# svg-project/Sparse-VideoGen

Hardware: AMD Instinct MI355X
Metric: attn_tflops_svg1_block_sparse (higher is better)
Workload: dtype bf16; 1 GPU; HunyuanVideo T2V hy720p SVG1 sparse layer-call: sample_mse(64 rows) + band attention with fused head placement, cfg=1 H=24 D=128 F=33 P=3600 ctx=256 prompt=64 S=119056 band=15616 density=0.2456; parallelism=single, variant=0, heads=alt

## Files before the change

### include/svg_attn.h

```cpp
#ifndef SVG_ATTN_H_
#define SVG_ATTN_H_

#include <stddef.h>
#include <stdint.h>

#ifdef __cplusplus
extern "C" {
#endif

#define SVG_DTYPE_BF16 0
#define SVG_DTYPE_F16 1
#define SVG_DTYPE_F32 2

#define SVG_OK 0
#define SVG_ERR_BAD_ARG (-1)
#define SVG_ERR_UNSUPPORTED (-2)
#define SVG_ERR_WORKSPACE (-3)
#define SVG_ERR_LAUNCH (-4)

#define SVG_ABI_VERSION 4
int svg_abi_version(void);

const char* svg_strerror(int code);
int svg_last_hip_error(void);
// ... 175 lines not shown
typedef struct svg_prologue_segment {
    const void* q_in;
    const void* k_in;
    const void* v_in;
    int32_t rows;
    int32_t norm_kind;
    const void* q_weight;
    const void* q_bias;
    const void* k_weight;
    const void* k_bias;
    float eps;
} svg_prologue_segment_t;

int svg_qk_norm_rope_transpose_joint(const svg_prologue_segment_t* seg, int32_t n_seg, void* q_out, void* k_out, void* v_out,
                                     int32_t bsz, int32_t H, int32_t D, int32_t dtype, int32_t rope_kind, const float* cos_or_real,
                                     const float* sin_or_imag, int32_t rope_lo, int32_t rope_hi, float q_scale, void* stream);

int svg_rmsnorm_rope_transpose(const void* q_in, const void* k_in, const void* v_in, void* q_out, void* k_out, void* v_out, int32_t bsz,
                               int32_t H, int32_t S, int32_t D, int32_t dtype, const void* q_weight, const void* k_weight,
                               int32_t w_dtype, float eps, int32_t rope_kind, const float* cos_or_real, const float* sin_or_imag,
                               int32_t rope_lo, int32_t rope_hi, float q_scale, void* stream);

int svg_layernorm_forward(const void* x, void* y, const void* weight, const void* bias, int64_t M, int32_t N, int32_t x_dtype,
                          int32_t y_dtype, int32_t w_dtype, float eps, void* stream);
int svg_modulate_shift_forward(const void* x, void* y, const float* scale, const float* shift, int64_t M, int32_t N,
                               int64_t rows_per_batch, int32_t x_dtype, int32_t y_dtype, void* stream);
int svg_modulate_gate_residual_forward(const void* residual, const void* x, const float* gate, void* y, int64_t M, int32_t N,
                                       int64_t rows_per_batch, int32_t r_dtype, int32_t x_dtype, int32_t y_dtype,
                                       void* stream);
int svg_layernorm_modulate_forward(const void* x, void* y, const void* weight, const void* bias, const float* scale,
                                   const float* shift, int64_t M, int32_t N, int64_t rows_per_batch, int32_t x_dtype,
                                   int32_t y_dtype, int32_t w_dtype, float eps, void* stream);
int svg_rmsnorm_forward(const void* x, void* y, const void* weight, int64_t M, int32_t N, int32_t x_dtype, int32_t y_dtype,
                        int32_t w_dtype, float eps, void* stream);
int svg_layernorm_forward_ex(const void* x, void* y, const void* weight, const void* bias, int64_t M, int32_t N, int32_t x_dtype,
                             int32_t y_dtype, int32_t w_dtype, float eps, int32_t reference_padding, void* stream);
int svg_layernorm_modulate_forward_ex(const void* x, void* y, const void* weight, const void* bias, const float* scale,
                                      const float* shift, int64_t M, int32_t N, int64_t rows_per_batch, int32_t x_dtype,
                                      int32_t y_dtype, int32_t w_dtype, float eps, int32_t reference_padding, void* stream);

int svg_band_attention_switch(const void* q, const void* k, const void* v, void* o, int32_t BH, int32_t S, int32_t D,
                              int32_t dtype, float sm_scale, const svg_band_mask_t* mask, const svg_perm_desc_t* perm,
                              const svg_band_mask_t* alt_mask, const int32_t* use_alt_flag, void* stream);
int svg_band_attention_switch_strided(const void* q, const void* k, const void* v, void* o, int32_t BH, int32_t S, int32_t D,
                                      int32_t dtype, float sm_scale, const svg_band_mask_t* mask, const svg_perm_desc_t* perm,
                                      const svg_band_mask_t* alt_mask, const int32_t* use_alt_flag,
                                      const svg_attn_layout_t* layout, void* stream);
int svg_sample_mse_flagged(const void* q, const void* k, const void* v, const int64_t* rows, int32_t R, int32_t BH, int32_t S,
                           int32_t D, int32_t dtype, float sm_scale, const svg_profile_desc_t* prof, float* out_mse,
                           void* workspace, size_t workspace_bytes, const int32_t* skip_flag, void* stream);

size_t svg_band_attention_fp8_workspace_bytes(int32_t BH, int32_t S, int32_t D);
int svg_band_attention_fp8(const void* q, const void* k, const void* v, void* o, int32_t BH, int32_t S, int32_t D, int32_t dtype,
                           float sm_scale, const svg_band_mask_t* mask, const svg_perm_desc_t* perm, void* workspace,
                           size_t workspace_bytes, void* stream);
int svg_band_attention_fp8_stage(const void* q, const void* k, const void* v, void* o, int32_t BH, int32_t S, int32_t D, int32_t dtype,
                                 float sm_scale, const svg_band_mask_t* mask, const svg_perm_desc_t* perm, void* workspace,
                                 size_t workspace_bytes, int32_t stage, void* stream);

size_t svg_varblock_attention_fp8_workspace_bytes(int32_t Hq, int32_t Hkv, int32_t QB, int32_t KB, int32_t Sq, int32_t Skv, int32_t D);
int svg_varblock_attention_fp8(const void* q, const void* k, const void* v, void* o, int32_t Hq, int32_t Hkv, int32_t Sq, int32_t Skv,
                               int32_t D, int32_t dtype, float sm_scale, const uint8_t* block_map, const int32_t* q_sizes,
                               const int32_t* k_sizes, int32_t QB, int32_t KB, const int32_t* q_row_idx, const int32_t* kv_row_idx,
                               void* workspace, size_t workspace_bytes, void* stream);

int32_t svg_band_attention_notify_target(int32_t S, const svg_band_mask_t* mask);
int svg_band_attention_notify(const void* q, const void* k, const void* v, void* o, int32_t BH, int32_t S, int32_t D,
                              int32_t dtype, float sm_scale, const svg_band_mask_t* mask, const svg_perm_desc_t* perm,
                              int32_t* done_per_head, int32_t done_words, void* stream);
int svg_wait_counters(const int32_t* counters, int32_t n, int32_t target, void* stream);
int svg_wait_counters_deadline(const int32_t* counters, int32_t n, int32_t target, int32_t timeout_ms, int32_t* timed_out,
                               void* stream);
int32_t svg_band_attention_notify_layout(int32_t S, const svg_band_mask_t* mask, int32_t nseg, int32_t* row_bounds, int32_t* targets);
int svg_band_attention_notify_seg(const void* q, const void* k, const void* v, void* o, int32_t BH, int32_t S, int32_t D,
                                  int32_t dtype, float sm_scale, const svg_band_mask_t* mask, const svg_perm_desc_t* perm,
                                  int32_t* done, int32_t done_words, int32_t nseg, void* stream);
int svg_band_attention_prescaled_notify_seg(const void* q_scaled, const void* k, const void* v, void* o, int32_t BH, int32_t S,
                                            int32_t D, int32_t dtype, const svg_band_mask_t* mask, const svg_perm_desc_t* perm,
                                            int32_t* done, int32_t done_words, int32_t nseg, void* stream);

int32_t svg_band_queue_order(int32_t BH, int32_t S, const svg_band_mask_t* mask, int32_t* out, int32_t out_words);
int svg_debug_band_queue_cap(int32_t max_workgroups);
int64_t svg_debug_band_replays(int32_t reset);

int svg_debug_pp_trace(uint64_t* out104);

int svg_debug_clock_probe(const int32_t* stop_flag, uint64_t* out2, int32_t max_ms, void* stream);

int svg_debug_wg_trace(uint64_t* out, int32_t n_workgroups);

#ifdef __cplusplus
}
#endif
#endif
```

### sparse-videogen_amd/csrc/attention.hip

```cpp
#include <algorithm>
#include <atomic>
#include <mutex>

#include "attn_core.h"
#include "attn_m16.h"
#include "band_policy.h"

namespace svg {

template <typename T, int D, int NW>
__global__ __launch_bounds__(NW * 64, 2) void band_attn_kernel(typename BandPolicy<T, D, NW>::Params prm) {
    extern __shared__ __attribute__((aligned(16))) char smem[];
    attn_body<T, D, NW, BandPolicy<T, D, NW>>(prm, smem, nullptr);
}

template <typename T, int D>
__global__ __launch_bounds__(512, (D == 64 ? 4 : 2)) void band_attn_pp2_kernel(typename BandPolicy<T, D, 8>::Params prm) {
    extern __shared__ __attribute__((aligned(16))) char smem[];
    attn_body_pp2<T, D, BandPolicy<T, D, 8>, false, 0, false, D == 64>(prm, smem, nullptr);
}
template <typename T>
__global__ __launch_bounds__(512, 4) void band_attn_pp2_switch64_kernel(typename BandPolicy<T, 64, 8>::Params prm,
                                                                        typename BandPolicy<T, 64, 8>::Params prm_alt,
                                                                        const int32_t* __restrict__ flag) {
// ... 370 lines not shown
extern "C" int svg_wait_counters(const int32_t* counters, int32_t n, int32_t target, void* stream) {
    if (!counters || n <= 0) return SVG_ERR_BAD_ARG;
    hipLaunchKernelGGL(wait_counters_kernel, dim3(1), dim3(64), 0, (hipStream_t)stream, counters, n, target);
    return launch_status();
}

extern "C" int svg_wait_counters_deadline(const int32_t* counters, int32_t n, int32_t target, int32_t timeout_ms,
                                          int32_t* timed_out, void* stream) {
    if (!counters || n <= 0 || timeout_ms <= 0 || !timed_out) return SVG_ERR_BAD_ARG;
    hipLaunchKernelGGL(wait_counters_deadline_kernel, dim3(1), dim3(64), 0, (hipStream_t)stream, counters, n, target,
                       (long long)timeout_ms * 100000LL, timed_out);
    return launch_status();
}

static BandOpts switch_opts(const svg_band_mask_t* alt_mask, const int32_t* use_alt_flag) {
    BandOpts opts;
    opts.alt_mask = alt_mask, opts.use_alt = use_alt_flag;
    return opts;
}

extern "C" int svg_band_attention_switch(const void* q, const void* k, const void* v, void* o, int32_t BH, int32_t S, int32_t D,
                                         int32_t dtype, float sm_scale, const svg_band_mask_t* mask, const svg_perm_desc_t* perm,
                                         const svg_band_mask_t* alt_mask, const int32_t* use_alt_flag, void* stream) {
    if (!alt_mask || !use_alt_flag) return SVG_ERR_BAD_ARG;
    return band_dispatch(q, k, v, o, BH, S, D, dtype, sm_scale, mask, perm, kBandAuto, switch_opts(alt_mask, use_alt_flag), 0, nullptr,
                         stream);
}

extern "C" int svg_band_attention_switch_strided(const void* q, const void* k, const void* v, void* o, int32_t BH, int32_t S, int32_t D,
                                                 int32_t dtype, float sm_scale, const svg_band_mask_t* mask, const svg_perm_desc_t* perm,
                                                 const svg_band_mask_t* alt_mask, const int32_t* use_alt_flag,
                                                 const svg_attn_layout_t* layout, void* stream) {
    if (!layout || !alt_mask || !use_alt_flag) return SVG_ERR_BAD_ARG;
    BandOpts opts = switch_opts(alt_mask, use_alt_flag);
    opts.strided = true;
    return band_dispatch(q, k, v, o, BH, S, D, dtype, sm_scale, mask, perm, kBandAuto, opts, 0, layout, stream);
}

extern "C" int svg_band_attention_switch_prescaled(const void* q_scaled, const void* k, const void* v, void* o, int32_t BH, int32_t S,
                                                   int32_t D, int32_t dtype, const svg_band_mask_t* mask, const svg_perm_desc_t* perm,
                                                   const svg_band_mask_t* alt_mask, const int32_t* use_alt_flag, void* stream) {
    if (!alt_mask || !use_alt_flag) return SVG_ERR_BAD_ARG;
    BandOpts opts = switch_opts(alt_mask, use_alt_flag);
    opts.prescaled = true;
    return band_dispatch(q_scaled, k, v, o, BH, S, D, dtype, 1.f, mask, perm, kBandAuto, opts, 0, nullptr, stream);
}

extern "C" int32_t svg_band_queue_order(int32_t BH, int32_t S, const svg_band_mask_t* mask, int32_t* out, int32_t out_words) {
    if (!mask || BH <= 0 || S <= 0 || check_band_mask(S, mask, nullptr) != SVG_OK) return -1;
    using Pol = svg::BandPolicy<__bf16, 128, 8>;
    const auto p = svg::make_band_params<Pol, __bf16>(nullptr, nullptr, nullptr, nullptr, BH, S, 1.f, mask, nullptr);
    const BandQueue qd = svg::make_band_queue<Pol>(p);
    if (!out) return qd.n_items;
    int n = 0;
    for (int x = 0; x <= kNumXCD; ++x)
        for (unsigned i = 0;; ++i) {
            const int w = x < kNumXCD ? qd.item(x, i) : qd.tail_item(i);
            if (w < 0) break;
            if (3 * (n + 1) > out_words) return -1;
            int head, qt;
            qd.decode(w, head, qt);
            Pol::Ctx c;
            Pol::kv_schedule(p, c, qt);
            out[3 * n] = x, out[3 * n + 1] = head * p.nqt + qt, out[3 * n + 2] = c.nT;
            ++n;
        }
    return n;
}

extern "C" int svg_debug_band_queue_cap(int32_t max_workgroups) {
    if (max_workgroups < 0) return SVG_ERR_BAD_ARG;
    g_queue_cap.store(max_workgroups, std::memory_order_relaxed);
    return SVG_OK;
}

extern "C" int64_t svg_debug_band_replays(int32_t reset) {
    unsigned n = 0;
    if (hipDeviceSynchronize() != hipSuccess || hipMemcpyFromSymbol(&n, HIP_SYMBOL(g_band_replays), sizeof n) != hipSuccess) return -1;
    const unsigned zero = 0;
    if (reset && hipMemcpyToSymbol(HIP_SYMBOL(g_band_replays), &zero, sizeof zero) != hipSuccess) return -1;
    return (int64_t)n;
}

extern "C" int svg_debug_wg_trace(uint64_t* out, int n_workgroups) { return g_trace_reader(out, true, n_workgroups); }
extern "C" int svg_debug_pp_trace(uint64_t* out104) { return g_trace_reader(out104, false, 0); }
```

### sparse-videogen_amd/csrc/attn_m16.h

```cpp
#pragma once
#include "attn_core.h"

namespace svg {

template <typename T>
struct Mfma16;
template <>
struct Mfma16<__bf16> {
    static __device__ __forceinline__ f32x4 mfma(bf16x8 a, bf16x8 b, f32x4 c) { return __builtin_amdgcn_mfma_f32_16x16x32_bf16(a, b, c, 0, 0, 0); }
    static __device__ __forceinline__ f32x4 mfma_keep_c(bf16x8 a, bf16x8 b, const f32x4& c) {
        f32x4 d;
        asm volatile("v_mfma_f32_16x16x32_bf16 %0, %1, %2, %3" : "=&v"(d) : "v"(a), "v"(b), "v"(c));
        return d;
    }
};
template <>
struct Mfma16<_Float16> {
    static __device__ __forceinline__ f32x4 mfma(f16x8 a, f16x8 b, f32x4 c) { return __builtin_amdgcn_mfma_f32_16x16x32_f16(a, b, c, 0, 0, 0); }
    static __device__ __forceinline__ f32x4 mfma_keep_c(f16x8 a, f16x8 b, const f32x4& c) {
        f32x4 d;
        asm volatile("v_mfma_f32_16x16x32_f16 %0, %1, %2, %3" : "=&v"(d) : "v"(a), "v"(b), "v"(c));
        return d;
    }
};

constexpr int attn_m16_lds_bytes() { return attn_pp2_lds_bytes<128>(); }

template <int D>
struct KvImage16 {
    static constexpr int kImg = kBN * D * 2, kStage = 2 * kImg;
    static constexpr unsigned col_v(int lane) {
        return ((lane & 3) ^ ((unsigned)((lane >> 4) & 1) << 1)) * 16u;
    }
    static constexpr unsigned col_k(int lane) { return col_v(lane); }
    static constexpr int k_lane(int g4, int n16) { return (n16 << 6) | ((g4 ^ (((n16 >> 2) & 1) << 1)) << 4); }
    static constexpr int v_lane0(int g4, int n16) { return kImg + (4 * g4 + (n16 >> 2)) * 64 + (((g4 & 1) * 16) + 4 * (n16 & 3)) * 2; }
    static constexpr int k_off(int k_lane, int kblk, int ks) { return k_lane + ks * (kBN * 64) + kblk * 1024; }
    static constexpr int v_off(int v_lane0, int v_lane1, int kc, int db, int h) {
        return ((db & 1) ? v_lane1 : v_lane0) + (db >> 1) * (kBN * 64) + (32 * kc + 16 * h) * 64;
    }
    static __device__ __forceinline__ i16x8 kfrag(const char* st, int k_lane, int kblk, int ks) {
        return *(const i16x8*)(st + k_off(k_lane, kblk, ks));
    }
    static __device__ __forceinline__ i16x8 vfrag(const char* st, int v_lane0, int v_lane1, int kc, int db) {
        return lds_read_tr16x2(st + v_off(v_lane0, v_lane1, kc, db, 0), st + v_off(v_lane0, v_lane1, kc, db, 1));
    }
    static constexpr int k_read(int key, int c) { return k_off(k_lane(c & 3, key & 15), key >> 4, c >> 2); }
    static constexpr int v_read(int key, int d) {
        const int lane = 16 * ((key >> 2) & 3) + (d & 15), src = tr16_src_lane(lane, key & 3), vl0 = v_lane0(src >> 4, src & 15);
        return v_off(vl0, vl0 ^ 32, key >> 5, d >> 4, (key >> 4) & 1) + 2 * (lane & 3);
    }
};
static_assert(kv_image_consistent<KvImage16<64>, 64>() && kv_image_consistent<KvImage16<128>, 128>(),
              "KvImage16: DMA columns and fragment reads disagree");

__device__ __forceinline__ float quad_group_max(float x) {
    x = vmax2(x, __shfl_xor(x, 16));
    return vmax2(x, __shfl_xor(x, 32));
}
__device__ __forceinline__ float quad_group_sum(float x) {
    x += __shfl_xor(x, 16);
    return x + __shfl_xor(x, 32);
}

template <typename P, typename = void>
struct HasAddOnStore : std::false_type {};
template <typename P>
struct HasAddOnStore<P, std::void_t<decltype(&P::add_on_store)>> : std::true_type {};

template <typename T>
__device__ __forceinline__ u32x2 add_rounded16(u32x2 a, u32x2 b) {
    using E = Elt<T>;
    const typename E::v4 x = __builtin_bit_cast(typename E::v4, a), y = __builtin_bit_cast(typename E::v4, b);
    typename E::v4 s;
#pragma unroll
    for (int j = 0; j < 4; ++j) s[j] = E::from_float(E::to_float(x[j]) + E::to_float(y[j]));
    return __builtin_bit_cast(u32x2, s);
}

constexpr int kCheckEvery = 8;
template <typename T, typename P, bool TRACE = false, int ONEBAR = -1, bool PRE = false, bool SPEC = false>
__device__ __forceinline__ bool attn_m16_tile(const typename P::Params& prm, const typename P::Ctx& ctx, char* smem,
                                              int check_mask = kCheckEvery - 1, unsigned* replay_ctr = nullptr) {
    using E = Elt<T>;
    using M = Mfma16<T>;
    using V8 = typename E::v8;
    constexpr int D = 128;
    constexpr int NW = 8;
    constexpr int KS = D / 32;
    constexpr int NDB = D / 16;
    using Img = KvImage16<D>;
    constexpr int NS = 4;
    constexpr int kImg = Img::kImg, kStage = Img::kStage;
    constexpr int NP = 2;
    constexpr int kCarry = 8;
    constexpr int kPF = 8;
    constexpr bool kOneBar = ONEBAR < 0 ? P::kOneBarrier : (ONEBAR != 0);
    static_assert(P::kRowBlocks == 1 && !P::kPartialOut && !P::kFixup && P::kIntervalMask, "band / variable-block policy");
    constexpr bool MSUM = std::is_same_v<T, __bf16> && !PRE;
    constexpr float kBias = MSUM ? 10.f : 0.f;
    constexpr bool kSpec = SPEC && MSUM;
    static_assert(!(SPEC && TRACE) && (kCheckEvery & (kCheckEvery - 1)) == 0, "SPEC: product kernels; a power of two");

    unsigned long long wg_t0 = 0, wg_t2 = 0;
    if constexpr (TRACE) wg_t0 = __builtin_amdgcn_s_memtime();
    const int tid = threadIdx.x;
    const int lane = tid & 63;
    const int wave = wave_id();
    const int g4 = lane >> 4;
    const int n16 = lane & 15;
    const bool lagging = wave >= NW / 2;
    const int nT = ctx.nT;
    volatile int* const spec_word = (volatile int*)(smem + attn_m16_lds_bytes() + 8);

    const T* __restrict__ qb = P::q_base(prm, ctx);
    const T* __restrict__ kb_ = P::k_base(prm, ctx);
    const T* __restrict__ vb = P::v_base(prm, ctx);
    const unsigned lds0 = (unsigned)(size_t)smem;

    const int dma_kg = wave / 2;
    const int dma_db0 = (wave % 2) * NP;
    const int krow = 16 * dma_kg + (lane >> 2);
    typename P::KvCursor cur;
    P::kv_cursor_init(prm, ctx, cur, krow);
    const unsigned col_v = (unsigned)(dma_db0 * 64 + Img::col_v(lane));
    const unsigned lds_piece = lds0 + (unsigned)(dma_db0 * (kBN * 64) + dma_kg * 1024);
    int nphys = 0, nnext = 0;
    auto resolve = [&](int t, auto guard_c) {
        if constexpr (decltype(guard_c)::value) nnext = (t < nT) ? P::kv_phys(prm, ctx, cur, t, krow) : 0;
        else nnext = P::kv_phys(prm, ctx, cur, t, krow);
    };
    constexpr std::true_type kGuarded{};
    auto take = [&]() { nphys = nnext; };
    const unsigned k_rsb = (unsigned)P::k_rs(prm) * 2u, v_rsb = (unsigned)P::v_rs(prm) * 2u;
    auto dma_piece = [&](int t, auto j_c) {
        constexpr int j = decltype(j_c)::value;
        const unsigned st = __builtin_amdgcn_readfirstlane(lds_piece + (unsigned)((t % NS) * kStage) + j * (kBN * 64));
        const unsigned ko = __umul24((unsigned)nphys, k_rsb) + col_v;
        const unsigned vo = __umul24((unsigned)nphys, v_rsb) + col_v;
        lds_dma16_kv<kImg>(st, ko, vo, (const char*)kb_ + j * 64, (const char*)vb + j * 64);
    };
    auto dma_issue = [&](int t) {
        dma_piece(t, std::integral_constant<int, 0>{});
        dma_piece(t, std::integral_constant<int, 1>{});
    };
    const int dist = lagging ? 3 : 2;
    for (int t = 0; t < dist; ++t) {
        resolve(t, kGuarded);
        take();
        if (t < nT) dma_issue(t);
    }
    resolve(dist, kGuarded);

    int q_log[2];
    V8 qf[2][KS];
    int m_a0[2], m_b0[2];
    unsigned m_alen[2], m_blen[2];
#pragma unroll
    for (int rb = 0; rb < 2; ++rb) {
        const int row_in_wg = wave * 32 + rb * 16 + n16;
        const int qp = P::q_phys(prm, ctx, row_in_wg);
        q_log[rb] = P::q_logical(ctx, row_in_wg);
        const T* qrow = qb + (size_t)(qp >= 0 ? qp : 0) * P::q_rs(prm) + g4 * 8;
#pragma unroll
        for (int ks = 0; ks < KS; ++ks) qf[rb][ks] = *(const V8*)(qrow + ks * 32);
        P::row_intervals(prm, ctx, q_log[rb], m_a0[rb], m_alen[rb], m_b0[rb], m_blen[rb]);
    }

    const int k_lane = Img::k_lane(g4, n16);
    const int v_lane0 = Img::v_lane0(g4, n16);
    const int v_lane1 = v_lane0 ^ 32;

    float m_run[2] = {-INFINITY, -INFINITY}, m_use[2] = {0.f, 0.f}, l_run[2] = {0.f, 0.f}, psum[2] = {0.f, 0.f};
    float m_sub[2] = {kBias, kBias};
    f32x4 acc_l[2] = {{0.f, 0.f, 0.f, 0.f}, {0.f, 0.f, 0.f, 0.f}};
    V8 ones8;
#pragma unroll
    for (int j = 0; j < 8; ++j) ones8[j] = E::from_float(1.f);
    bool force_exact = true;
    int spec_mode = -1;
    f32x4 acc_o[NDB][2];
#pragma unroll
    for (int db = 0; db < NDB; ++db)
#pragma unroll
        for (int rb = 0; rb < 2; ++rb)
#pragma unroll
            for (int r = 0; r < 4; ++r) acc_o[db][rb][r] = 0.f;
    const float c_log2 = prm.scale_log2;
    if constexpr (MSUM) asm volatile("" : "+v"(ones8));

#pragma unroll
    for (int rb = 0; rb < 2; ++rb)
#pragma unroll
        for (int ks = 0; ks < KS; ++ks) asm volatile("" : "+v"(qf[rb][ks]));
    asm volatile("s_waitcnt vmcnt(0)" ::: "memory");
    pp_barrier();
    if (!kOneBar && lagging) pp_barrier();

    const bool idle = !P::wave_active(ctx, wave * 32);

    unsigned tr_acc[4] = {0, 0, 0, 0};
    unsigned long long tr_last = 0, tr_first = 0;
    if constexpr (TRACE) tr_first = tr_last = __builtin_amdgcn_s_memtime();
    auto tick = [&](auto slot_c) {
        if constexpr (TRACE) {
            constexpr int slot = decltype(slot_c)::value;
            const unsigned long long now = __builtin_amdgcn_s_memtime();
            tr_acc[slot] += (unsigned)(now - tr_last);
            tr_last = now;
        }
    };

    f32x4 neg_ref[2] = {{0.f, 0.f, 0.f, 0.f}, {0.f, 0.f, 0.f, 0.f}};
    float pre_shift[2] = {0.f, 0.f};
    f32x4 sc[4][2];
    V8 pf[2][2];
    float psum_thr = -1.f;

    auto kfrag = [&](const char* st, int kblk, int ks) -> i16x8 { return Img::kfrag(st, k_lane, kblk, ks); };
    auto vfrag = [&](const char* st, int kc, int db) -> i16x8 { return Img::vfrag(st, v_lane0, v_lane1, kc, db); };
    auto probs_impl = [&](int kc, auto shifted_c) {
        constexpr bool shifted = decltype(shifted_c)::value;
// ... 162 lines not shown
            }
        };
#pragma unroll
        for (int i = kCarry; i < kPF; ++i) fetch(i);
        __builtin_amdgcn_sched_barrier(0);
#pragma unroll
        for (int i = 0; i < NALL; ++i) {
            fetch(i + kPF);
            if constexpr (has_next) {
                if (i + kPF >= NALL && i + kPF - NALL < kCarry) carry_load(t + 1, i + kPF - NALL);
            }
            if (i < NPV) {
                const int kc = i / NDB, db = i % NDB;
                const V8 a = __builtin_bit_cast(V8, i < kCarry ? carry[i < kCarry ? i : 0] : ring[i % (kPF + 1)]);
                acc_o[db][0] = M::mfma(a, pf[kc][0], acc_o[db][0]);
                acc_o[db][1] = M::mfma(a, pf[kc][1], acc_o[db][1]);
                if constexpr (MSUM) {
                    if (db == kMsumAt) {
                        acc_l[0] = M::mfma(ones8, pf[kc][0], acc_l[0]);
                        acc_l[1] = M::mfma(ones8, pf[kc][1], acc_l[1]);
                    }
                } else {
                    if (i == NPV - 1) l_run[0] += psum[0], l_run[1] += psum[1];
                }
            } else {
                const int j = i - NPV, ks = j >> 2, b = j & 3;
                const V8 a = __builtin_bit_cast(V8, ring[i % (kPF + 1)]);
                if constexpr (PRE) {
                    sc[b][0] = ks == 0 ? M::mfma_keep_c(a, qf[0][ks], neg_ref[0]) : M::mfma(a, qf[0][ks], sc[b][0]);
                    sc[b][1] = ks == 0 ? M::mfma_keep_c(a, qf[1][ks], neg_ref[1]) : M::mfma(a, qf[1][ks], sc[b][1]);
                } else {
                    sc[b][0] = M::mfma(a, qf[0][ks], ks == 0 ? zero : sc[b][0]);
                    sc[b][1] = M::mfma(a, qf[1][ks], ks == 0 ? zero : sc[b][1]);
                }
            }
            __builtin_amdgcn_sched_barrier(0);
        }
        if constexpr (has_next) {
#pragma unroll
            for (int b = 0; b < 4; ++b) asm volatile("" : "+v"(sc[b][0]), "+v"(sc[b][1]));
        }
    };

    auto spec_replay = [&](bool bad) -> bool {
        if (__any(bad) && lane == 0) *spec_word = 1;
        pp_barrier();
        if (__builtin_amdgcn_readfirstlane(*spec_word) == 0) return false;
        if (replay_ctr && tid == 0) atomicAdd(replay_ctr, 1u);
        return true;
    };

    if (idle) {
        for (int t = 0; t < nT; ++t) {
            if (!kOneBar || lagging) pp_barrier();
            stage_resolve_next(t, kGuarded);
            stage_request(t);
            if (!kOneBar || !lagging) pp_barrier();
        }
        pp_barrier();
        if (!kOneBar && !lagging) pp_barrier();
        if constexpr (kSpec) {
            if (check_mask != 0 && spec_replay(false)) return true;
        }
        P::notify(prm, ctx);
        return false;
    }

    if (nT > 0) {
        const f32x4 zero = {0.f, 0.f, 0.f, 0.f};
#pragma unroll
        for (int ks = 0; ks < KS; ++ks)
#pragma unroll
            for (int b = 0; b < 4; ++b) {
                const V8 a = __builtin_bit_cast(V8, kfrag(smem, b, ks));
                sc[b][0] = M::mfma(a, qf[0][ks], ks == 0 ? zero : sc[b][0]);
                sc[b][1] = M::mfma(a, qf[1][ks], ks == 0 ? zero : sc[b][1]);
            }
#pragma unroll
        for (int b = 0; b < 4; ++b) asm volatile("" : "+v"(sc[b][0]), "+v"(sc[b][1]));
#pragma unroll
        for (int i = 0; i < kCarry; ++i) carry_load(0, i);
    }
    const int bar_n = lagging ? 1 : 0, bar_m = lagging ? 0 : 1;
    auto tile = [&](int t, auto has_next_c, auto guard_c) {
        tick(std::integral_constant<int, 0>{});
        if constexpr (kOneBar) pp_barrier_if(bar_n);
        else pp_barrier();
        tick(std::integral_constant<int, 1>{});
        vector_phase(t, guard_c);
        tick(std::integral_constant<int, 2>{});
        if constexpr (kOneBar) pp_barrier_if(bar_m);
        else pp_barrier();
        tick(std::integral_constant<int, 3>{});
        __builtin_amdgcn_s_setprio(1);
        matrix_phase(t, has_next_c);
        __builtin_amdgcn_s_setprio(0);
    };
    int t = 0;
    for (const int n_main = nT - dist - 1; t < n_main; ++t) tile(t, std::true_type{}, std::false_type{});
    for (; t + 1 < nT; ++t) tile(t, std::true_type{}, kGuarded);
    if (nT > 0) tile(nT - 1, std::false_type{}, kGuarded);
    pp_barrier();
    if (!kOneBar && !lagging) pp_barrier();
    if constexpr (TRACE) {
        if (blockIdx.x == kPpTraceBlock && lane == 0) {
#pragma unroll
            for (int j = 0; j < 4; ++j) g_pp_trace[wave * 8 + j] = tr_acc[j];
            if (wave == 0) g_pp_trace[64] = (unsigned long long)nT, g_pp_trace[65] = tr_last - tr_first;
        }
        wg_t2 = __builtin_amdgcn_s_memtime();
    }
    if constexpr (kSpec) {
        if (check_mask != 0) {
            bool bad = !(fabsf(acc_l[0][0]) < 0x1p120f) || !(fabsf(acc_l[1][0]) < 0x1p120f);
#pragma unroll
            for (int db = 0; db < NDB; ++db)
#pragma unroll
                for (int rb = 0; rb < 2; ++rb)
#pragma unroll
                    for (int r = 0; r < 4; ++r) bad = bad || !(fabsf(acc_o[db][rb][r]) < 0x1p120f);
            if (spec_replay(bad)) return true;
        }
    }

    constexpr int kEpiStride = D * 2 + 8;
    char* erow = smem + (size_t)(wave * 32) * kEpiStride;
#pragma unroll
    for (int rb = 0; rb < 2; ++rb) {
        const float l_tot = MSUM ? acc_l[rb][0] : quad_group_sum(l_run[rb]);
        const float inv = l_tot > 0.f ? 1.f / l_tot : 0.f;
#pragma unroll
        for (int db = 0; db < NDB; ++db) {
            typename E::v4 o4;
#pragma unroll
            for (int j = 0; j < 4; ++j) o4[j] = E::from_float(acc_o[db][rb][j] * inv);
            *(typename E::v4*)(erow + (rb * 16 + n16) * kEpiStride + (16 * db + 4 * g4) * 2) = o4;
        }
    }
    __builtin_amdgcn_s_waitcnt(0xc07f);
    __builtin_amdgcn_wave_barrier();
    T* __restrict__ ob = P::o_base(prm, ctx);
    const int o_rs = P::o_rs(prm);
    constexpr int kLanesPerRow = D * 2 / 8;
    constexpr int kRowsPerPass = 64 / kLanesPerRow;
    const int sub = lane / kLanesPerRow;
    const int colb = (lane - sub * kLanesPerRow) * 8;
    int ephys[32 / kRowsPerPass];
#pragma unroll
    for (int i = 0; i < 32 / kRowsPerPass; ++i) ephys[i] = P::q_phys(prm, ctx, wave * 32 + i * kRowsPerPass + sub);
#pragma unroll
    for (int i = 0; i < 32 / kRowsPerPass; ++i) {
        const int rr = i * kRowsPerPass + sub;
        u32x2 val = *(const u32x2*)(erow + rr * kEpiStride + colb);
        if (ephys[i] >= 0) {
            u32x2* const dst = (u32x2*)((char*)(ob + (size_t)ephys[i] * o_rs) + colb);
            if constexpr (HasAddOnStore<P>::value) {
                if (P::add_on_store(prm)) val = add_rounded16<T>(*dst, val);
            }
            *dst = val;
        }
    }
    P::notify(prm, ctx);
    if constexpr (TRACE) {
        asm volatile("s_waitcnt vmcnt(0)" ::: "memory");
        if (wave == 0 && lane == 0 && blockIdx.x < (unsigned)kWgTraceMax) {
            unsigned long long* w = g_wg_trace + (size_t)blockIdx.x * 6;
            w[0] = wg_t0, w[1] = tr_first, w[2] = wg_t2, w[3] = __builtin_amdgcn_s_memtime();
            w[4] = __builtin_amdgcn_s_getreg((31 << 11) | 4);
            w[5] = __builtin_amdgcn_s_getreg((31 << 11) | 20);
        }
    }
    return false;
}

// ... 16 lines not shown
```

### sparse-videogen_amd/csrc/band_policy.h

```cpp
#pragma once
#include <algorithm>

#include "attn_core.h"

namespace svg {

struct BandOpts {
    int32_t* done = nullptr;
    int done_nseg = 1;
    bool prescaled = false;
    bool trace = false;
    int trace_abl = 0;
    bool strided = false;
    AttnLayout lay{};
    const svg_band_mask_t* alt_mask = nullptr;
    const int32_t* use_alt = nullptr;
};

inline int check_band_mask(int S, const svg_band_mask_t* mask, const svg_perm_desc_t* perm) {
    if (mask->real_len < 0 || mask->real_len > S || mask->band < 0 || mask->band > S + 1) return SVG_ERR_BAD_ARG;
    if (mask->colfull_lo > mask->colfull_hi || mask->rowfull_lo > mask->rowfull_hi) return SVG_ERR_BAD_ARG;
    if (perm && perm->head_perm_flag) {
        if (perm->num_frame <= 0 || perm->frame_size <= 0 || perm->vid0 < 0 ||
            (int64_t)perm->vid0 + (int64_t)perm->num_frame * perm->frame_size > S)
// ... 159 lines not shown
    static __device__ __forceinline__ void tile_cur_shift(TileCur& tc) {
        tc.k0 = tc.k1, tc.left = tc.left1;
        tc.k1 = tc.k2, tc.left1 = tc.left2;
        tc.left2 = 0;
    }
    static __device__ __forceinline__ void tile_cur_init(const Ctx& c, TileCur& tc) {
        tc.k0 = c.seg_lo[0] * kBN, tc.left = c.seg_n[0];
        tc.k1 = c.seg_lo[1] * kBN, tc.left1 = c.seg_n[1];
        tc.k2 = c.seg_lo[2] * kBN, tc.left2 = c.seg_n[2];
        if (tc.left <= 0) tile_cur_shift(tc);
        if (tc.left <= 0) tile_cur_shift(tc);
    }
    static __device__ __forceinline__ void tile_cur_next(const Ctx& c, TileCur& tc) {
        tile_cur_step(tc);
        if (tile_cur_ended(tc)) tile_cur_fix(c, tc);
    }
    static __device__ __forceinline__ void tile_cur_step(TileCur& tc) {
        tc.k0 += kBN;
        --tc.left;
    }
    static __device__ __forceinline__ bool tile_cur_ended(const TileCur& tc) { return tc.left <= 0; }
    static __device__ __forceinline__ void tile_cur_fix(const Ctx&, TileCur& tc) {
        tile_cur_shift(tc);
        if (tc.left <= 0) tile_cur_shift(tc);
    }
    static constexpr bool kRowStep = true;
    struct RowState {
        int l, f, physv;
    };
    static __device__ __forceinline__ void rows_seek(const Params& p, const Ctx& c, RowState& st, int k0, int row) {
        st.l = k0 + row;
        const int i = st.l - p.vid0;
        const int a = i >= 0 ? i : -i - 1;
        const int qd = (int)((unsigned)a / (unsigned)p.F);
        const int pp = i >= 0 ? qd : -qd - 1;
        st.f = i - pp * p.F;
        st.physv = p.vid0 + st.f * p.P + pp;
    }
    static __device__ __forceinline__ void rows_step(const Params& p, const Ctx&, RowState& st) {
        st.l += kBN;
        int f = st.f + p.r64, physv = st.physv + p.sp64;
        const bool wrap = f >= p.F;
        st.f = wrap ? f - p.F : f;
        st.physv = wrap ? physv + p.wrap_phys : physv;
    }
    static __device__ __forceinline__ int rows_phys(const Params& p, const Ctx& c, const RowState& st) {
        const bool in_video = (unsigned)(st.l - p.vid0) < (unsigned)p.V;
        const int phys = (c.perm && in_video) ? st.physv : st.l;
        return st.l < p.S ? phys : 0;
    }
    static __device__ __forceinline__ bool fast_full(const Ctx& c, int k0) { return k0 >= c.fk_lo && k0 <= c.fk_hi; }
    static __device__ __forceinline__ void kv_cursor_init(const Params&, const Ctx&, KvCursor& cu, int) {
        cu.physv = 0, cu.f = 0, cu.prev_k0 = -(1 << 30);
    }
    static __device__ __forceinline__ int kv_phys(const Params& p, const Ctx& c, KvCursor& cu, int t, int row) {
        return kv_phys_at(p, c, cu, tile_key0(c, t), row);
    }
    static __device__ __forceinline__ int kv_phys_at(const Params& p, const Ctx& c, KvCursor& cu, int k0, int row) {
        const int l = k0 + row;
        if (!c.perm) return l < p.S ? l : 0;
        int f, physv;
        const int delta = __builtin_amdgcn_readfirstlane(k0 - cu.prev_k0);
        if (delta == kBN) {
            f = cu.f + p.r64;
            physv = cu.physv + p.sp64;
            const bool wrap = f >= p.F;
            f = wrap ? f - p.F : f;
            physv = wrap ? physv + p.wrap_phys : physv;
        } else {
            const int i = l - p.vid0;
            const int a = i >= 0 ? i : -i - 1;
            const int qd = (int)((unsigned)a / (unsigned)p.F);
            const int pp = i >= 0 ? qd : -qd - 1;
            f = i - pp * p.F;
            physv = p.vid0 + f * p.P + pp;
        }
        cu.physv = physv, cu.f = f, cu.prev_k0 = k0;
        if (k0 >= p.vid0 && k0 + kBN <= p.vid0 + p.V) return physv;
        const bool in_video = (unsigned)(l - p.vid0) < (unsigned)p.V;
        const int phys = in_video ? physv : l;
        return l < p.S ? phys : 0;
    }

    static __device__ __forceinline__ int classify(const Params& p, const Ctx& c, int k0, int wrow0) {
        if (k0 >= c.fk_lo && k0 <= c.fk_hi) return TILE_FULL;
        const int w0 = c.q0 + wrow0;
        if (w0 >= c.q_end) return TILE_SKIP;
        const int w1 = min(w0 + kWR, c.q_end);
        const int k1 = min(k0 + kBN, p.S);
        const int real = p.real_len;
        bool all = false;
        if (k0 + kBN <= p.S) {
            if (w1 <= real && k1 <= real) {
                const bool band_all = (k1 - 1 - w0 < p.band) && (w1 - 1 - k0 < p.band);
                const bool col_all = (k0 >= p.cf_lo && k1 <= p.cf_hi);
                const bool row_all = (w0 >= p.rf_lo && w1 <= p.rf_hi);
                all = band_all || col_all || row_all;
            } else if (w0 >= real && k0 >= real) {
                all = true;
            }
        }
        if (all) return TILE_FULL;
        bool any = false;
        if (w0 < real && k0 < real) {
            const int w1r = min(w1, real), k1r = min(k1, real);
            const bool band_any = (k0 - (w1r - 1) < p.band) && (w0 - (k1r - 1) < p.band);
            const bool col_any = (k0 < p.cf_hi && k1r > p.cf_lo);
            const bool row_any = (w0 < p.rf_hi && w1r > p.rf_lo);
            any = band_any || col_any || row_any;
        }
        if (w1 > real && k1 > real) any = true;
        return any ? TILE_PARTIAL : TILE_SKIP;
    }
    static __device__ __forceinline__ bool allowed(const Params& p, const Ctx&, int q, int k) {
        const bool rq = q < p.real_len, rk = k < p.real_len;
        const bool in_band = (p.band > 0) & ((unsigned)(q - k + p.band - 1) < (unsigned)(2 * p.band - 1));
        const bool colf = (unsigned)(k - p.cf_lo) < (unsigned)(p.cf_hi - p.cf_lo);
        const bool rowf = (unsigned)(q - p.rf_lo) < (unsigned)(p.rf_hi - p.rf_lo);
        return ((rq & rk) & (in_band | colf | rowf)) | ((!rq & !rk) & (k < p.S));
    }
    static __device__ __forceinline__ void row_intervals(const Params& p, const Ctx&, int q, int& a0, unsigned& alen, int& b0,
                                                         unsigned& blen) {
        const int real = p.real_len;
        const bool rq = q < real;
        const bool rowf = (unsigned)(q - p.rf_lo) < (unsigned)(p.rf_hi - p.rf_lo);
        const int band_lo = max(q - p.band + 1, 0), band_hi = min(q + p.band, real);
        const int lo = rq ? (rowf ? 0 : band_lo) : real;
        const int hi = rq ? (rowf ? real : band_hi) : p.S;
        a0 = lo, alen = (unsigned)max(hi - lo, 0);
        const int ch = min(p.cf_hi, real);
        b0 = p.cf_lo, blen = (rq && !rowf) ? (unsigned)max(ch - p.cf_lo, 0) : 0u;
    }
    static __device__ __forceinline__ float score_fixup(const Params&, float s) { return s; }
    static __device__ __forceinline__ void notify(const Params& p, const Ctx& c) {
        if (p.done) {
            asm volatile("s_waitcnt vmcnt(0)" ::: "memory");
            __threadfence();
            if ((threadIdx.x & 63) == 0) {
                int32_t* cnt = p.done + c.head * p.done_nseg;
                if (!c.perm) {
                    atomicAdd(cnt + min(c.qt / p.done_tps, p.done_nseg - 1), 1);
                } else if (atomicAdd(p.done + p.BH * p.done_nseg + c.head, 1) == p.nqt * NW - 1) {
                    __threadfence();
                    for (int sgm = 0; sgm < p.done_nseg; ++sgm) {
                        const int t_lo = sgm * p.done_tps;
                        const int t_hi = (sgm == p.done_nseg - 1) ? p.nqt : min(p.nqt, (sgm + 1) * p.done_tps);
                        atomicAdd(cnt + sgm, (t_hi - t_lo) * NW);
                    }
                }
            }
        }
    }
};

constexpr int kQueueChunk = 32;
constexpr int kQueueTail = 256;
constexpr int kQueueStride = 16;
constexpr int kQueueCounters = kNumXCD + 2;
constexpr int kQueueWords = kQueueCounters * kQueueStride;

struct BandQueue {
    int32_t* ctr;
    int n_items;
    int BH, nh, n_heavy, heavy_lo;
    int nl;
    int e_lo, e_hi;
// ... 153 lines not shown
```

### sparse-videogen_amd/svg/_native.py

```python
from __future__ import annotations

import ctypes as C
import os
from pathlib import Path
from typing import NamedTuple, Optional, Sequence

import torch

_LIB_PATH = Path(__file__).resolve().parent.parent / "lib" / "libsvgattn.so"
_lib: Optional[C.CDLL] = None
_load_error: Optional[str] = None

SVG_DTYPE_BF16, SVG_DTYPE_F16 = 0, 1


class BandMask(C.Structure):

    _fields_ = [
        ("real_len", C.c_int32),
        ("band", C.c_int32),
        ("colfull_lo", C.c_int32),
        ("colfull_hi", C.c_int32),
        ("rowfull_lo", C.c_int32),
        ("rowfull_hi", C.c_int32),
    ]

    def as_tuple(self):
        return (self.real_len, self.band, self.colfull_lo, self.colfull_hi, self.rowfull_lo, self.rowfull_hi)


class PermDesc(C.Structure):

    _fields_ = [
        ("head_perm_flag", C.c_void_p),
        ("vid0", C.c_int32),
        ("num_frame", C.c_int32),
        ("frame_size", C.c_int32),
    ]


class ProfileVariant(C.Structure):

    _fields_ = [
        ("coord", C.c_int32),
        ("origin", C.c_int32),
        ("span", C.c_int32),
        ("band_blocks", C.c_int32),
        ("sink_cols", C.c_int32),
        ("text_lo", C.c_int32),
        ("text_hi", C.c_int32),
    ]


class ProfileDesc(C.Structure):

    _fields_ = [
        ("vid0", C.c_int32),
        ("num_frame", C.c_int32),
        ("frame_size", C.c_int32),
        ("emulate_bf16", C.c_int32),
        ("variant", ProfileVariant * 2),
    ]


_I32, _I64, _F32, _VP, _SZ = C.c_int32, C.c_int64, C.c_float, C.c_void_p, C.c_size_t


class PrologueSegment(C.Structure):
    _fields_ = [("q_in", C.c_void_p), ("k_in", C.c_void_p), ("v_in", C.c_void_p), ("rows", C.c_int32), ("norm_kind", C.c_int32),
                ("q_weight", C.c_void_p), ("q_bias", C.c_void_p), ("k_weight", C.c_void_p), ("k_bias", C.c_void_p), ("eps", C.c_float)]


class TensorStrides(C.Structure):
    _fields_ = [("batch", C.c_int64), ("head", C.c_int64), ("row", C.c_int64)]


class AttnLayout(C.Structure):
    _fields_ = [("heads_per_batch", C.c_int32), ("kv_heads_per_batch", C.c_int32), ("q", TensorStrides), ("k", TensorStrides),
                ("v", TensorStrides), ("o", TensorStrides)]


SIGNATURES = {
    "svg_abi_version": (C.c_int, []),
    "svg_strerror": (C.c_char_p, [C.c_int]),
    "svg_last_hip_error": (C.c_int, []),
    "svg_build_info": (C.c_char_p, []),
    "svg_debug_pp_trace": (C.c_int, [_VP]),
    "svg_debug_wg_trace": (C.c_int, [_VP, _I32]),
    "svg_band_queue_order": (_I32, [_I32, _I32, C.POINTER(BandMask), _VP, _I32]),
    "svg_debug_band_queue_cap": (C.c_int, [_I32]),
    "svg_debug_band_replays": (C.c_int64, [_I32]),
    "svg_rms_norm_forward": (C.c_int, [_VP, _VP, C.c_int64, _I32, _I32, C.c_float, _VP]),
    "svg_layer_norm_forward": (C.c_int, [_VP, _VP, _VP, C.c_int64, _I32, _I32, _VP]),
    "svg_apply_qk_rope_inplace_cossin": (C.c_int, [_VP, _VP, _VP, _VP, _I32, _I32, _I32, _I32, _I32, _I32, _I32, _VP]),
    "svg_apply_qk_rope_inplace_cossin_txtlast": (C.c_int, [_VP, _VP, _VP, _VP, _I32, _I32, _I32, _I32, _I32, _I32, _I32, _VP]),
    "svg_apply_qk_rope_inplace_cossin_complex": (C.c_int, [_VP, _VP, _VP, _VP, _I32, _I32, _I32, _I32, _I32, _I32, _I32, _VP]),
    "svg_bsr_to_block_map": (C.c_int, [_VP, _VP, _I32, _I32, _I32, _I32, _I32, _I32, _VP, _VP, _VP, _VP]),
    "svg_layernorm_forward": (C.c_int, [_VP, _VP, _VP, _VP, C.c_int64, _I32, _I32, _I32, _I32, C.c_float, _VP]),
    "svg_rmsnorm_forward": (C.c_int, [_VP, _VP, _VP, C.c_int64, _I32, _I32, _I32, _I32, C.c_float, _VP]),
    "svg_layernorm_forward_ex": (C.c_int, [_VP, _VP, _VP, _VP, C.c_int64, _I32, _I32, _I32, _I32, C.c_float, _I32, _VP]),
    "svg_modulate_shift_forward": (C.c_int, [_VP, _VP, _VP, _VP, C.c_int64, _I32, C.c_int64, _I32, _I32, _VP]),
    "svg_modulate_gate_residual_forward": (C.c_int, [_VP, _VP, _VP, _VP, C.c_int64, _I32, C.c_int64, _I32, _I32, _I32, _VP]),
    "svg_layernorm_modulate_forward": (C.c_int, [_VP, _VP, _VP, _VP, _VP, _VP, C.c_int64, _I32, C.c_int64, _I32, _I32, _I32,
                                                 C.c_float, _VP]),
    "svg_layernorm_modulate_forward_ex": (C.c_int, [_VP, _VP, _VP, _VP, _VP, _VP, C.c_int64, _I32, C.c_int64, _I32, _I32, _I32,
                                                    C.c_float, _I32, _VP]),
    "svg_qk_norm_rope_transpose": (C.c_int, [_VP, _VP, _VP, _VP, _I32, _I32, _I32, _I32, _I32, _I32, _I32, _VP, _VP, _VP, _VP,
                                             C.c_float, _I32, _VP, _VP, _I32, _I32, _VP]),
    "svg_qk_norm_rope": (C.c_int, [_VP, _VP, _I32, _I32, _I32, _I32, _I32, _I32, _I32, _VP, _VP, _VP, _VP, C.c_float, _I32, _VP,
                                   _VP, _I32, _I32, _VP]),
    "svg_qk_norm_rope_qscale": (C.c_int, [_VP, _VP, _I32, _I32, _I32, _I32, _I32, _I32, _I32, _VP, _VP, _VP, _VP, C.c_float, _I32, _VP,
                                          _VP, _I32, _I32, C.c_float, _VP]),
    "svg_qk_norm_rope_transpose_qscale": (C.c_int, [_VP, _VP, _VP, _VP, _I32, _I32, _I32, _I32, _I32, _I32, _I32, _VP, _VP, _VP, _VP,
                                                    C.c_float, _I32, _VP, _VP, _I32, _I32, C.c_float, _VP]),
    "svg_qk_norm_rope_transpose_joint": (C.c_int, [C.POINTER(PrologueSegment), _I32, _VP, _VP, _VP, _I32, _I32, _I32, _I32, _I32, _VP, _VP,
                                                   _I32, _I32, C.c_float, _VP]),
    "svg_rmsnorm_rope_transpose": (C.c_int, [_VP, _VP, _VP, _VP, _VP, _VP, _I32, _I32, _I32, _I32, _I32, _VP, _VP, _I32, C.c_float, _I32, _VP,
                                             _VP, _I32, _I32, C.c_float, _VP]),
    "svg_head_placement": (C.c_int, [_VP, _VP, _I32, _VP, _I32, _I32, _I32, _I32, _I32, _I32, _I32, _I32, _I32, _VP]),
    "svg_permute_rows": (C.c_int, [_VP, _VP, _VP, _I32, _I32, _I32, _I32, _VP]),
    "svg_inverse_permute_rows": (C.c_int, [_VP, _VP, _VP, _I32, _I32, _I32, _I32, _VP]),
    "svg_argsort_workspace_bytes": (_SZ, [_I32, _I32, _I32]),
    "svg_argsort_labels": (C.c_int, [_VP, _VP, _VP, _I32, _I32, _I32, _VP, _SZ, _VP]),
    "svg_band_attention": (C.c_int, [_VP, _VP, _VP, _VP, _I32, _I32, _I32, _I32, _F32, C.POINTER(BandMask),
                                     C.POINTER(PermDesc), _I32, _VP]),
    "svg_band_attention_strided": (C.c_int, [_VP, _VP, _VP, _VP, _I32, _I32, _I32, _I32, _F32, C.POINTER(BandMask),
                                             C.POINTER(PermDesc), C.POINTER(AttnLayout), _VP]),
    "svg_band_attention_switch_strided": (C.c_int, [_VP, _VP, _VP, _VP, _I32, _I32, _I32, _I32, _F32, C.POINTER(BandMask),
                                                    C.POINTER(PermDesc), C.POINTER(BandMask), _VP, C.POINTER(AttnLayout), _VP]),
    "svg_varblock_attention_strided": (C.c_int, [_VP, _VP, _VP, _VP, _I32, _I32, _I32, _I32, _I32, _I32, _F32, _VP, _VP, _VP,
                                                 _I32, _I32, _VP, _VP, _VP, _SZ, C.POINTER(AttnLayout), _VP]),
    "svg_cross_attention": (C.c_int, [_VP, _VP, _VP, _VP, _I32, _I32, _I32, _I32, _I32, _F32, C.POINTER(AttnLayout), _VP]),
    "svg_cross_attention_keyrange": (C.c_int, [_VP, _VP, _VP, _VP, _I32, _I32, _I32, _I32, _I32, _F32, _VP, _VP, _I32, C.POINTER(AttnLayout),
                                               _VP]),
    "svg_cross_attention_pair": (C.c_int, [_VP, _VP, _VP, _VP, _VP, _VP, _I32, _I32, _I32, _I32, _I32, _I32, _F32, C.POINTER(AttnLayout),
                                           C.POINTER(AttnLayout), _VP]),
    "svg_sample_mse_strided": (C.c_int, [_VP, _VP, _VP, _VP, _I32, _I32, _I32, _I32, _I32, _F32, C.POINTER(ProfileDesc), _VP, _VP,
                                         _SZ, _VP, C.POINTER(AttnLayout), _VP]),
    "svg_band_attention_prescaled": (C.c_int, [_VP, _VP, _VP, _VP, _I32, _I32, _I32, _I32, C.POINTER(BandMask), C.POINTER(PermDesc), _VP]),
    "svg_band_attention_switch_prescaled": (C.c_int, [_VP, _VP, _VP, _VP, _I32, _I32, _I32, _I32, C.POINTER(BandMask),
                                                      C.POINTER(PermDesc), C.POINTER(BandMask), _VP, _VP]),
    "svg_debug_clock_probe": (C.c_int, [_VP, _VP, _I32, _VP]),
    "svg_band_attention_prescaled_notify_seg": (C.c_int, [_VP, _VP, _VP, _VP, _I32, _I32, _I32, _I32, C.POINTER(BandMask),
                                                          C.POINTER(PermDesc), _VP, _I32, _I32, _VP]),
    "svg_band_attention_notify_target": (_I32, [_I32, C.POINTER(BandMask)]),
    "svg_band_attention_notify": (C.c_int, [_VP, _VP, _VP, _VP, _I32, _I32, _I32, _I32, _F32, C.POINTER(BandMask),
                                            C.POINTER(PermDesc), _VP, _I32, _VP]),
    "svg_varblock_attention_fp8_workspace_bytes": (_SZ, [_I32, _I32, _I32, _I32, _I32, _I32, _I32]),
    "svg_varblock_attention_fp8": (C.c_int, [_VP, _VP, _VP, _VP, _I32, _I32, _I32, _I32, _I32, _I32, _F32, _VP, _VP, _VP, _I32, _I32,
                                             _VP, _VP, _VP, _SZ, _VP]),
    "svg_band_attention_fp8_workspace_bytes": (_SZ, [_I32, _I32, _I32]),
    "svg_band_attention_fp8": (C.c_int, [_VP, _VP, _VP, _VP, _I32, _I32, _I32, _I32, _F32, _VP, _VP, _VP, _SZ, _VP]),
    "svg_band_attention_fp8_stage": (C.c_int, [_VP, _VP, _VP, _VP, _I32, _I32, _I32, _I32, _F32, _VP, _VP, _VP, _SZ, _I32, _VP]),
    "svg_wait_counters": (C.c_int, [_VP, _I32, _I32, _VP]),
    "svg_wait_counters_deadline": (C.c_int, [_VP, _I32, _I32, _I32, _VP, _VP]),
    "svg_band_attention_notify_layout": (_I32, [_I32, C.POINTER(BandMask), _I32, _VP, _VP]),
    "svg_band_attention_notify_seg": (C.c_int, [_VP, _VP, _VP, _VP, _I32, _I32, _I32, _I32, _F32, C.POINTER(BandMask),
                                                C.POINTER(PermDesc), _VP, _I32, _I32, _VP]),
    "svg_band_attention_switch": (C.c_int, [_VP, _VP, _VP, _VP, _I32, _I32, _I32, _I32, _F32, C.POINTER(BandMask),
                                            C.POINTER(PermDesc), C.POINTER(BandMask), _VP, _VP]),
    "svg_sample_mse_flagged": (C.c_int, [_VP, _VP, _VP, _VP, _I32, _I32, _I32, _I32, _I32, _F32, C.POINTER(ProfileDesc), _VP, _VP,
                                         _SZ, _VP, _VP]),
    "svg_varblock_workspace_bytes": (_SZ, [_I32, _I32, _I32, _I32, _I32]),
    "svg_varblock_attention": (C.c_int, [_VP, _VP, _VP, _VP, _I32, _I32, _I32, _I32, _I32, _I32, _F32, _VP, _VP, _VP,
                                         _I32, _I32, _VP, _VP, _VP, _SZ, _I32, _VP]),
    "svg_sample_mse_workspace_bytes": (_SZ, [_I32, _I32, _I32, _I32]),
    "svg_sample_mse": (C.c_int, [_VP, _VP, _VP, _VP, _I32, _I32, _I32, _I32, _I32, _F32, C.POINTER(ProfileDesc), _VP, _VP,
                                 _SZ, _VP]),
    "svg_kmeans_xsq": (C.c_int, [_VP, _VP, _I32, _I32, _I32, _I32, _VP]),
    "svg_kmeans_workspace_bytes": (_SZ, [_I32, _I32, _I32, _I32]),
    "svg_kmeans_iter": (C.c_int, [_VP, _VP, _VP, _VP, _VP, _VP, _VP, _VP, _I32, _I32, _I32, _I32, _I32, _VP, _SZ, _VP]),
    "svg_kmeans_assign": (C.c_int, [_VP, _VP, _VP, _I32, _I32, _I32, _I32, _I32, _VP, _SZ, _VP]),
    "svg_kmeans_update": (C.c_int, [_VP, _VP, _VP, _VP, _VP, _VP, _VP, _I32, _I32, _I32, _I32, _I32, _VP, _SZ, _VP]),
    "svg_kmeans_loop_workspace_bytes": (_SZ, [_I32, _I32, _I32, _I32]),
# ... 1030 lines not shown
```

Baseline: 1346 TFLOP/s.

## Replace per-tile KV permutation index math with incremental row-walk cursor

Adds a RowWalk cursor to the band policy. It advances each DMA row's physical KV index by a precomputed stride with a wrap correction when consecutive tiles are contiguous, and falls back to the exact divide-based permutation mapping only otherwise. The kernel also computes the K/V byte offsets once at take time instead of on every DMA piece. The one-barrier pipeline now uses a scalar-flag branch barrier. The aim is to cut VALU work and integer division from the address-generation path, at the cost of more complex cursor state, extra registers and a host debug entry point for validation.

```diff
diff --git a/include/svg_attn.h b/include/svg_attn.h
--- a/include/svg_attn.h
+++ b/include/svg_attn.h
@@ -281,6 +281,8 @@
 int32_t svg_band_queue_order(int32_t BH, int32_t S, const svg_band_mask_t* mask, int32_t* out, int32_t out_words);
 int svg_debug_band_queue_cap(int32_t max_workgroups);
 int64_t svg_debug_band_replays(int32_t reset);
+int32_t svg_debug_band_row_cursor(int32_t S, int32_t vid0, int32_t num_frame, int32_t frame_size, int32_t token_major,
+                                  const int32_t* k0, int32_t n, int32_t* out, int32_t out_words, int32_t* cheap);
 
 int svg_debug_pp_trace(uint64_t* out104);
 
diff --git a/sparse-videogen_amd/csrc/attention.hip b/sparse-videogen_amd/csrc/attention.hip
--- a/sparse-videogen_amd/csrc/attention.hip
+++ b/sparse-videogen_amd/csrc/attention.hip
@@ -476,5 +476,30 @@
     return (int64_t)n;
 }
 
+extern "C" int32_t svg_debug_band_row_cursor(int32_t S, int32_t vid0, int32_t num_frame, int32_t frame_size, int32_t token_major,
+                                             const int32_t* k0, int32_t n, int32_t* out, int32_t out_words, int32_t* cheap) {
+    using Pol = svg::BandPolicy<__bf16, 128, 8>;
+    if (S <= 0 || n < 0 || !k0 || !out || (int64_t)out_words < (int64_t)n * kBN) return -1;
+    const svg_band_mask_t mask{S, S, 0, 0, 0, 0};
+    const int64_t flag = 1;
+    const svg_perm_desc_t perm{&flag, vid0, num_frame, frame_size};
+    if (check_band_mask(S, &mask, &perm) != SVG_OK) return -1;
+    const Pol::Params p = svg::make_band_params<Pol, __bf16>(nullptr, nullptr, nullptr, nullptr, 1, S, 1.f, &mask, &perm);
+    Pol::Ctx c{};
+    c.perm = token_major != 0;
+    for (int row = 0; row < kBN; ++row) {
+        Pol::RowWalk w;
+        Pol::row_walk_init(p, c, w);
+        int phys = 0;
+        for (int i = 0; i < n; ++i) {
+            Pol::RowWalk probe = w;
+            if (cheap) cheap[i] = Pol::row_walk_cheap(probe, k0[i]) ? 1 : 0;
+            Pol::row_walk_next(p, w, phys, k0[i], row);
+            out[(size_t)i * kBN + row] = phys;
+        }
+    }
+    return n;
+}
+
 extern "C" int svg_debug_wg_trace(uint64_t* out, int n_workgroups) { return g_trace_reader(out, true, n_workgroups); }
 extern "C" int svg_debug_pp_trace(uint64_t* out104) { return g_trace_reader(out104, false, 0); }
diff --git a/sparse-videogen_amd/csrc/attn_m16.h b/sparse-videogen_amd/csrc/attn_m16.h
--- a/sparse-videogen_amd/csrc/attn_m16.h
+++ b/sparse-videogen_amd/csrc/attn_m16.h
@@ -67,6 +67,19 @@
 struct HasAddOnStore : std::false_type {};
 template <typename P>
 struct HasAddOnStore<P, std::void_t<decltype(&P::add_on_store)>> : std::true_type {};
+
+template <typename P, typename = void>
+struct HasRowCursor : std::false_type {};
+template <typename P>
+struct HasRowCursor<P, std::void_t<decltype(P::kRowCursor)>> : std::true_type {};
+
+template <bool when_set>
+__device__ __forceinline__ void pp_barrier_sel(int flag) {
+    __builtin_amdgcn_sched_barrier(0);
+    if constexpr (when_set) asm volatile("s_cmp_eq_u32 %0, 0\n\ts_cbranch_scc1 1f\n\ts_waitcnt lgkmcnt(0)\n\ts_barrier\n1:" ::"s"(flag) : "memory", "scc");
+    else asm volatile("s_cmp_lg_u32 %0, 0\n\ts_cbranch_scc1 1f\n\ts_waitcnt lgkmcnt(0)\n\ts_barrier\n1:" ::"s"(flag) : "memory", "scc");
+    __builtin_amdgcn_sched_barrier(0);
+}
 
 template <typename T>
 __device__ __forceinline__ u32x2 add_rounded16(u32x2 a, u32x2 b) {
@@ -121,23 +134,47 @@
     const int dma_kg = wave / 2;
     const int dma_db0 = (wave % 2) * NP;
     const int krow = 16 * dma_kg + (lane >> 2);
-    typename P::KvCursor cur;
-    P::kv_cursor_init(prm, ctx, cur, krow);
+    constexpr bool kCursor = HasRowCursor<P>::value;
+    auto cur = [&] {
+        if constexpr (kCursor) {
+            typename P::RowWalk w;
+            P::row_walk_init(prm, ctx, w);
+            return w;
+        } else {
+            typename P::KvCursor c;
+            P::kv_cursor_init(prm, ctx, c, krow);
+            return c;
+        }
+    }();
     const unsigned col_v = (unsigned)(dma_db0 * 64 + Img::col_v(lane));
     const unsigned lds_piece = lds0 + (unsigned)(dma_db0 * (kBN * 64) + dma_kg * 1024);
+    const unsigned k_rsb = (unsigned)P::k_rs(prm) * 2u, v_rsb = (unsigned)P::v_rs(prm) * 2u;
     int nphys = 0, nnext = 0;
+    unsigned req_ko = 0, req_vo = 0;
     auto resolve = [&](int t, auto guard_c) {
-        if constexpr (decltype(guard_c)::value) nnext = (t < nT) ? P::kv_phys(prm, ctx, cur, t, krow) : 0;
-        else nnext = P::kv_phys(prm, ctx, cur, t, krow);
+        if constexpr (kCursor) {
+            if (!decltype(guard_c)::value || t < nT) P::row_walk_next(prm, cur, nnext, P::tile_key0(ctx, t), krow);
+        } else if constexpr (decltype(guard_c)::value) {
+            nnext = (t < nT) ? P::kv_phys(prm, ctx, cur, t, krow) : 0;
+        } else {
+            nnext = P::kv_phys(prm, ctx, cur, t, krow);
+        }
     };
     constexpr std::true_type kGuarded{};
-    auto take = [&]() { nphys = nnext; };
-    const unsigned k_rsb = (unsigned)P::k_rs(prm) * 2u, v_rsb = (unsigned)P::v_rs(prm) * 2u;
+    auto take = [&]() {
+        if constexpr (kCursor) {
+            req_ko = __umul24((unsigned)nnext, k_rsb) + col_v;
+            req_vo = __umul24((unsigned)nnext, v_rsb) + col_v;
+            asm volatile("" : "+v"(req_ko), "+v"(req_vo));
+        } else {
+            nphys = nnext;
+        }
+    };
     auto dma_piece = [&](int t, auto j_c) {
         constexpr int j = decltype(j_c)::value;
         const unsigned st = __builtin_amdgcn_readfirstlane(lds_piece + (unsigned)((t % NS) * kStage) + j * (kBN * 64));
-        const unsigned ko = __umul24((unsigned)nphys, k_rsb) + col_v;
-        const unsigned vo = __umul24((unsigned)nphys, v_rsb) + col_v;
+        const unsigned ko = kCursor ? req_ko : __umul24((unsigned)nphys, k_rsb) + col_v;
+        const unsigned vo = kCursor ? req_vo : __umul24((unsigned)nphys, v_rsb) + col_v;
         lds_dma16_kv<kImg>(st, ko, vo, (const char*)kb_ + j * 64, (const char*)vb + j * 64);
     };
     auto dma_issue = [&](int t) {
@@ -466,14 +503,17 @@
         for (int i = 0; i < kCarry; ++i) carry_load(0, i);
     }
     const int bar_n = lagging ? 1 : 0, bar_m = lagging ? 0 : 1;
+    const int lag_s = __builtin_amdgcn_readfirstlane(bar_n);
     auto tile = [&](int t, auto has_next_c, auto guard_c) {
         tick(std::integral_constant<int, 0>{});
-        if constexpr (kOneBar) pp_barrier_if(bar_n);
+        if constexpr (kOneBar && kCursor) pp_barrier_sel<true>(lag_s);
+        else if constexpr (kOneBar) pp_barrier_if(bar_n);
         else pp_barrier();
         tick(std::integral_constant<int, 1>{});
         vector_phase(t, guard_c);
         tick(std::integral_constant<int, 2>{});
-        if constexpr (kOneBar) pp_barrier_if(bar_m);
+        if constexpr (kOneBar && kCursor) pp_barrier_sel<false>(lag_s);
+        else if constexpr (kOneBar) pp_barrier_if(bar_m);
         else pp_barrier();
         tick(std::integral_constant<int, 3>{});
         __builtin_amdgcn_s_setprio(1);
diff --git a/sparse-videogen_amd/csrc/band_policy.h b/sparse-videogen_amd/csrc/band_policy.h
--- a/sparse-videogen_amd/csrc/band_policy.h
+++ b/sparse-videogen_amd/csrc/band_policy.h
@@ -265,6 +265,64 @@
         return l < p.S ? phys : 0;
     }
 
+    static constexpr bool kRowCursor = true;
+    struct RowWalk {
+        int perm, lo, hi;
+        int step, end, unwrap;
+        int vlen;
+        int prev_k0;
+    };
+    static __host__ __device__ __forceinline__ void row_walk_init(const Params& p, const Ctx& c, RowWalk& w) {
+        const bool perm = c.perm != 0;
+        w.perm = perm;
+        w.lo = perm ? p.vid0 + kBN : -(1 << 30);
+        w.hi = (perm ? p.vid0 + p.V : p.S) - kBN;
+        w.step = perm ? p.sp64 : kBN, w.end = p.vid0 + p.V, w.unwrap = 1 - p.V;
+        w.vlen = perm ? p.V : 0;
+        w.prev_k0 = -(1 << 30);
+#ifdef __HIP_DEVICE_COMPILE__
+        asm volatile("" : "+v"(w.step), "+v"(w.unwrap));
+        w.perm = __builtin_amdgcn_readfirstlane(w.perm);
+        asm volatile("" : "+s"(w.perm));
+#endif
+    }
+    static __host__ __device__ __forceinline__ bool row_walk_cheap(RowWalk& w, int k0) {
+        const bool cheap = (k0 == w.prev_k0 + kBN) & (k0 >= w.lo) & (k0 <= w.hi);
+        w.prev_k0 = k0;
+        return cheap;
+    }
+    static __host__ __device__ __forceinline__ void row_add(int& phys, int d) {
+#ifdef __HIP_DEVICE_COMPILE__
+        asm("v_add_u32 %0, %0, %1" : "+v"(phys) : "v"(d));
+#else
+        phys += d;
+#endif
+    }
+    static __host__ __device__ __forceinline__ void row_set(int& phys, int x) {
+#ifdef __HIP_DEVICE_COMPILE__
+        asm("v_mov_b32 %0, %1" : "+v"(phys) : "v"(x));
+#else
+        phys = x;
+#endif
+    }
+    static __host__ __device__ __forceinline__ int row_exact(const Params& p, int vlen, int l) {
+        const int i = l - p.vid0;
+        const int a = i >= 0 ? i : -i - 1;
+        const int qd = (int)((unsigned)a / (unsigned)p.F);
+        const int pp = i >= 0 ? qd : -qd - 1;
+        const int f = i - pp * p.F;
+        const int physv = p.vid0 + f * p.P + pp;
+        const bool in_video = (unsigned)i < (unsigned)vlen;
+        const int phys = in_video ? physv : l;
+        return l < p.S ? phys : 0;
+    }
+    static __host__ __device__ __forceinline__ void row_walk_next(const Params& p, RowWalk& w, int& phys, int k0, int row) {
+        const bool cheap = row_walk_cheap(w, k0);
+        row_add(phys, w.step);
+        if (w.perm) row_add(phys, phys >= w.end ? w.unwrap : 0);
+        if (__builtin_expect(!cheap, 0)) row_set(phys, row_exact(p, w.vlen, k0 + row));
+    }
+
     static __device__ __forceinline__ int classify(const Params& p, const Ctx& c, int k0, int wrow0) {
         if (k0 >= c.fk_lo && k0 <= c.fk_hi) return TILE_FULL;
         const int w0 = c.q0 + wrow0;
diff --git a/sparse-videogen_amd/svg/_native.py b/sparse-videogen_amd/svg/_native.py
--- a/sparse-videogen_amd/svg/_native.py
+++ b/sparse-videogen_amd/svg/_native.py
@@ -90,6 +90,7 @@
     "svg_band_queue_order": (_I32, [_I32, _I32, C.POINTER(BandMask), _VP, _I32]),
     "svg_debug_band_queue_cap": (C.c_int, [_I32]),
     "svg_debug_band_replays": (C.c_int64, [_I32]),
+    "svg_debug_band_row_cursor": (_I32, [_I32, _I32, _I32, _I32, _I32, _VP, _I32, _VP, _I32, _VP]),
     "svg_rms_norm_forward": (C.c_int, [_VP, _VP, C.c_int64, _I32, _I32, C.c_float, _VP]),
     "svg_layer_norm_forward": (C.c_int, [_VP, _VP, _VP, C.c_int64, _I32, _I32, _VP]),
     "svg_apply_qk_rope_inplace_cossin": (C.c_int, [_VP, _VP, _VP, _VP, _I32, _I32, _I32, _I32, _I32, _I32, _I32, _VP]),
```

Result: faster. 1374 TFLOP/s, median of 6 (+2.1%).
